# aszepieniec/stark-anatomy

Hardware: AMD Instinct MI355X
Metric: ntt_field_elements_per_sec (higher is better)
Workload: dtype u128; 1 GPU; ntt_fwd_inv_2^20_1gpu; log2n=20, parallelism=single, passes_per_transform=2

## Files before the change

### include/starkcore.h

```cpp
#ifndef STARKCORE_H
#define STARKCORE_H
#include <stdint.h>

#ifdef __cplusplus
extern "C" {
#endif

#define SC_OK 0
#define SC_ERR_HIP (-1)
#define SC_ERR_NOT_POW2 (-2)
#define SC_ERR_ROOT_ORDER (-3)
#define SC_ERR_ROOT_NOT_PRIMITIVE (-4)
#define SC_ERR_DIV_ZERO (-5)
#define SC_ERR_BAD_ARG (-6)
#define SC_ERR_UNSUPPORTED (-7)
#define SC_ERR_NOT_INIT (-8)
#define SC_ERR_TIMEOUT (-9)

typedef struct sc_vec sc_vec_t;
typedef struct sc_merkle sc_merkle_t;
typedef struct sc_merkle_forest sc_merkle_forest_t;
typedef struct sc_later sc_later_t;
typedef struct sc_polytree sc_polytree_t;
typedef struct sc_geodomain sc_geodomain_t;

int sc_device_count(void);
int sc_init(int device);
int sc_shutdown(void);
const char* sc_last_error(void);
int sc_synchronize(void);
int sc_stream(void** stream_out);
int sc_stream_join(void* other_stream);
int sc_set_tuning(const char* key, int value);
int sc_ntt_num_passes(uint64_t n);
int sc_debug_trace(void* d_buf);

int sc_field_selftest(int op, const void* a, const void* b, void* out, uint64_t n);
int sc_field_selftest2(int op, const void* a, const void* b, const void* c, const void* d, void* out, uint32_t* word, uint64_t n);

int sc_vec_alloc(uint64_t n, sc_vec_t** out);
int sc_vec_free(sc_vec_t* v);
int sc_vec_wrap(void* d_elems, uint64_t n, sc_vec_t** out);
uint64_t sc_vec_len(const sc_vec_t* v);
void* sc_vec_ptr(sc_vec_t* v);
int sc_vec_zero(sc_vec_t* v);
int sc_vec_upload(sc_vec_t* v, uint64_t offset, const void* host, uint64_t count);
int sc_vec_download(const sc_vec_t* v, uint64_t offset, void* host, uint64_t count);
int sc_vec_gather(const sc_vec_t* v, const uint64_t* indices, uint64_t k, void* host_out);
int sc_memcpy_dev(void* d_dst, const void* d_src, uint64_t count, void* stream);

int sc_ntt(const void* in, void* out, uint64_t n, const uint64_t root[2], int inverse);
int sc_ntt_dev(const void* d_in, void* d_out, uint64_t n, const uint64_t root[2], int inverse, void* stream);
int sc_ntt_columns_dev(const void* d_in, void* d_out, uint64_t n, uint64_t cols, const uint64_t root[2], int inverse, void* stream);

int sc_ntt_batch_dev(const void* d_in, void* d_out, uint64_t len, uint64_t batch, int kind, const uint64_t root[2], void* stream);
int sc_ntt_batch_ex_dev(const void* d_in, void* d_out, uint64_t len, uint64_t batch, int kind, const uint64_t root[2],
                        const uint64_t outer_root[2], uint64_t outer_order, uint64_t outer_col_base, int outer_scale_ninv, uint64_t chunks, void* stream);
int sc_ntt_rows_t_ld_dev(const void* d_in, void* d_out, uint64_t len, uint64_t batch, const uint64_t root[2], uint64_t chunks, uint64_t out_ld, void* stream);
typedef struct sc_fourstep sc_fourstep_t;
typedef struct { char internal[128]; } sc_rccl_id_t;
int sc_fourstep_create(int log2n, const uint64_t root[2], int rank, int world, sc_fourstep_t** plan);
int sc_fourstep_create_ex(int log2n, const uint64_t root[2], int rank, int world, int log_n1, sc_fourstep_t** plan);
int sc_fourstep_free(sc_fourstep_t* plan);
int sc_fourstep_shape(const sc_fourstep_t* plan, int inverse, uint64_t* rows, uint64_t* cols_total);
int sc_fourstep_cols_dev(const sc_fourstep_t* plan, int inverse, const void* d_src, void* d_send, void* d_recv_diag, void* stream);
int sc_fourstep_rows_dev(const sc_fourstep_t* plan, int inverse, const void* d_recv, void* d_dst, uint64_t block, uint64_t nblocks, int defer_last_pass, void* stream);
int sc_fourstep_rows_finish_dev(const sc_fourstep_t* plan, int inverse, void* d_dst, void* stream);
int sc_comm_unique_id(const char* rccl_path, sc_rccl_id_t* id_out);
int sc_comm_init(const char* rccl_path, const sc_rccl_id_t* id, int rank, int world);
int sc_comm_destroy(void);
int sc_fourstep_run_dev(const sc_fourstep_t* plan, int inverse, const void* d_src, void* d_send, void* d_recv, void* d_dst, uint64_t nblocks, int defer_last_pass,
                        int force_diag_exchange, void* stream);
int sc_ipc_region_create(uint64_t bytes, void** d_region, uint8_t handle_out[64]);
int sc_ipc_region_create_ex(uint64_t bytes, int kind, void** d_region, uint8_t handle_out[64]);
int sc_ipc_region_kind(int* fine_grained);
int sc_ipc_region_open(const uint8_t handle[64], void** d_region);
int sc_ipc_region_close(void* d_region);
int sc_ipc_region_free(void* d_region);
int sc_fourstep_region_bytes(const sc_fourstep_t* plan, uint64_t* bytes);
int sc_fourstep_set_peers(sc_fourstep_t* plan, void* const* regions);
int sc_fourstep_run_direct_dev(sc_fourstep_t* plan, int inverse, const void* d_src, void* d_dst, void* stream);
int sc_fourstep_direct_status(const sc_fourstep_t* plan, uint64_t* timed_out_epoch);
int sc_twiddle_matrix_dev(void* d_data, uint64_t rows, uint64_t cols, uint64_t row_base, uint64_t col_base, const uint64_t root[2], uint64_t order,
                          const uint64_t scale[2], void* stream);

int sc_coset_evaluate(const void* coeffs, uint64_t m, const uint64_t offset[2], const uint64_t generator[2], uint64_t order, void* out);
int sc_coset_evaluate_dev(const void* d_coeffs, uint64_t m, const uint64_t offset[2], const uint64_t generator[2], uint64_t order, void* d_out, void* stream);
// ... 130 lines not shown
```

### stark-anatomy_amd/csrc/core.h

```cpp
#pragma once
#include <hip/hip_runtime.h>
#include <dlfcn.h>
#include <cstdio>
#include <cstdlib>
#include <cstring>
#include <algorithm>
#include <atomic>
#include <chrono>
#include <cerrno>
#include <thread>
#include <sys/random.h>
#include <deque>
#include <functional>
#include <future>
#include <map>
#include <mutex>
#include <string>
#include <tuple>
#include <vector>

#pragma GCC visibility push(default)
#include "../../include/starkcore.h"
#pragma GCC visibility pop
#include "ntt_plan.h"
// ... 43 lines not shown

struct PlanKey {
    int logn;
    uint64_t lo, hi;
    bool operator<(const PlanKey& o) const { return std::tie(logn, lo, hi) < std::tie(o.logn, o.lo, o.hi); }
};
struct PlanTables {
    Fe* mt = nullptr;
    int mt_log = 0;
    Fe* tl = nullptr;
    Fe* th = nullptr;
    Fe* th_ninv = nullptr;
    struct Direct { int logA, logR; bool scaled; Fe* d; };
    std::vector<Direct> direct;
    uint64_t last_use = 0;
};
struct OuterKey {
    uint64_t lo, hi, order, len, batch, col_base;
    int ninv;
    bool operator<(const OuterKey& o) const { return std::tie(lo, hi, order, len, batch, col_base, ninv) < std::tie(o.lo, o.hi, o.order, o.len, o.batch, o.col_base, o.ninv); }
};
struct OuterTable {
    Fe* d = nullptr;
    uint64_t last_use = 0;
};
struct PowKey {
    uint64_t lo, hi, hi_count;
    bool operator<(const PowKey& o) const { return std::tie(lo, hi, hi_count) < std::tie(o.lo, o.hi, o.hi_count); }
};
struct PowTables {
    Fe* lo = nullptr;
    Fe* hi = nullptr;
    uint64_t last_use = 0;
};

struct Ctx {
    bool init = false;
    int device = -1;
    hipStream_t stream = nullptr;
    std::string err;
    NttTuning tuning;
    std::map<PlanKey, PlanTables> plans;
    std::map<PowKey, PowTables> pows;
    std::map<OuterKey, OuterTable> outers;
    uint64_t tick = 0;
    bool foreign_streams = false;
    int small_divisor_direct = 1;
    int div_cols_launch_log = 26;
    int div_cols_chunk = 0;
    std::vector<hipStream_t> seen_streams;
    DevBuf scratch[8];
    std::map<hipStream_t, DevBuf> ntt_work;
    std::map<hipStream_t, DevBuf> ntt_flags;
    int fast_fixups = 1;
    int num_cus = 256;
    int xcd_remap = 1;
    int fixed_shapes = 1;
    int prio_balance = -1;
    int wave_local = 1;
    unsigned long long* trace = nullptr;
    int forest_four_lane_wgs = 256;
    int merkle_big_nlev = 2;
    int fri_tail = -1;
    int fri_tail_stall = -1;
    size_t verify_stage_bytes = 64ull << 20;
    uint8_t* root_slots = nullptr;
    uint8_t* later_words = nullptr;
    uint64_t root_seq = 0;
    std::vector<int> free_root_slots;
};
constexpr int ROOT_SLOTS = 256;
constexpr size_t ROOT_SLOT_BYTES = 128;
constexpr size_t LATER_WORD_BYTES = 128;
constexpr long SPIN_POLLS = 40000000;

struct PendingFree {
    void* p;
    size_t bytes;
    std::vector<hipEvent_t> evs;
};
#define HIPCHK(expr)                                                                                          \
    do {                                                                                                      \
        hipError_t _e = (expr);                                                                               \
        if (_e != hipSuccess) return fail(SC_ERR_HIP, std::string(#expr) + ": " + hipGetErrorString(_e));     \
    } while (0)

#define SCCHK(expr)              \
    do {                         \
        int _rc = (expr);        \
        if (_rc != SC_OK) return _rc; \
    } while (0)

struct NttOpts {
    uint64_t in_limit = ~0ull;
    const PowTables* coset = nullptr;
    uint32_t cols = 1;
    uint64_t col_stride_in = 0;
};
constexpr uint64_t COLS_ELEMS_PER_LAUNCH = 1ull << 26;
constexpr uint64_t SMALL_DIVISOR = 8;

constexpr uint64_t FUSE_MAX_W = 1ull << 17;

enum BuildMode { BUILD_SYNC = 0, BUILD_ASYNC = 1, BUILD_NOROOT = 2 };

extern Ctx g;
// ... 129 lines not shown
```

### stark-anatomy_amd/csrc/core.hip

```cpp
#include "core.h"


template <int LOGE> struct PassThreads { static constexpr int value = LOGE >= 4 ? 256 : (LOGE == 3 ? 512 : 1024); };

template <int LOGE>
__global__ void __launch_bounds__(PassThreads<LOGE>::value) ntt_pass_kernel(const PassParams P, uint32_t ntiles, int xcd_remap) {
    extern __shared__ __attribute__((aligned(16))) unsigned char smem_raw[];
    Fe* lds = reinterpret_cast<Fe*>(smem_raw);
    uint32_t wg = blockIdx.x, colbits = 0;
    if (P.col_enable) { colbits = (wg >> P.col_tiles_log) << P.col_tiles_log; wg -= colbits; }
    uint32_t tile = wg;
    if (xcd_remap) tile = (wg & 7u) * (ntiles >> 3) + (wg >> 3);
    tile |= colbits;
    Fe* tw = lds + (1u << (P.logR + P.logC));
    tile_twiddles_to_lds(P, P.logR, threadIdx.x, blockDim.x, tw);
    __syncthreads();
    const int nrounds = (P.logR + LOGE - 1) / LOGE;
    int sh = P.logR;
    for (int r = 0; r < nrounds; ++r) {
        const int s = (r == 0) ? (P.logR - LOGE * (nrounds - 1)) : LOGE;
        sh -= s;
        ntt_round_dispatch<LOGE>(P, s, sh, r == 0, tile, threadIdx.x, lds, tw);
        if (r + 1 < nrounds) __syncthreads();
    }
// ... 8 lines not shown
    if constexpr (TRACE) {
        if (P.trace) {
            trow = P.trace + ((size_t)blockIdx.x * (blockDim.x >> 6) + (threadIdx.x >> 6)) * TRACE_STAMPS;
            if ((threadIdx.x & 63u) == 0) { trow[0] = __builtin_amdgcn_s_memtime(); trow[15] = __builtin_amdgcn_s_memrealtime(); }
        }
    }
    uint32_t wg = blockIdx.x, colbits = 0;
    if (P.col_enable) { colbits = (wg >> P.col_tiles_log) << P.col_tiles_log; wg -= colbits; }
    uint32_t tile = wg;
    if (xcd_remap) tile = (wg & 7u) * (ntiles >> 3) + (wg >> 3);
    tile |= colbits;
    Fe* tw = lds + (1u << (GLR + GLC));
    auto stamp = [&](int i) {
        if constexpr (TRACE) {
            if (trow) {
                if (i == 2) __builtin_amdgcn_s_waitcnt(0);
                if ((threadIdx.x & 63u) == 0 && i < 13) trow[i] = __builtin_amdgcn_s_memtime();
            }
        }
    };
    auto sync = [] { __syncthreads(); };
    auto wsync = [] { __builtin_amdgcn_fence(__ATOMIC_RELEASE, "wavefront"); __builtin_amdgcn_wave_barrier(); __builtin_amdgcn_fence(__ATOMIC_ACQUIRE, "wavefront"); };
    FixedRounds<LOGE, GLR, GLC, 0, ALT>::run(P, tile, threadIdx.x, lds, tw, sync, wsync, stamp, wave_local != 0);
    if constexpr (TRACE) {
        if (trow && (threadIdx.x & 63u) == 0) { __builtin_amdgcn_s_waitcnt(0); trow[14] = __builtin_amdgcn_s_memtime(); trow[13] = __builtin_amdgcn_s_memrealtime(); }
    }
}

template <int GLR, int GLC>
__device__ __forceinline__ uint32_t fixed8_tile(const PassParams& P, uint32_t index, uint32_t ntiles, int xcd_remap) {
    uint32_t wg = index, colbits = 0;
    if (P.col_enable) { colbits = (wg >> P.col_tiles_log) << P.col_tiles_log; wg -= colbits; }
    uint32_t tile = wg;
    if (xcd_remap) tile = (wg & 7u) * (ntiles >> 3) + (wg >> 3);
    return tile | colbits;
}
template <int GLR, int GLC>
__global__ void __launch_bounds__(1 << (GLR + GLC - 3)) __attribute__((amdgpu_waves_per_eu(4)))
ntt_pass_kernel_fixed8(const PassParams P, uint32_t ntiles, int xcd_remap, int wave_local, uint32_t* flags) {
    extern __shared__ __attribute__((aligned(16))) unsigned char smem_raw[];
    Fe* lds = reinterpret_cast<Fe*>(smem_raw);
    const uint32_t tile = fixed8_tile<GLR, GLC>(P, blockIdx.x, ntiles, xcd_remap);
    Fe* tw = lds + (1u << (GLR + GLC));
    auto stamp = [](int) {};
    auto sync = [] { __syncthreads(); };
    auto wsync = [] { __builtin_amdgcn_fence(__ATOMIC_RELEASE, "wavefront"); __builtin_amdgcn_wave_barrier(); __builtin_amdgcn_fence(__ATOMIC_ACQUIRE, "wavefront"); };
    rare_t rare = 0;
    FixedRounds<3, GLR, GLC, 0, false, true>::run(P, tile, threadIdx.x, lds, tw, sync, wsync, stamp, wave_local != 0, rare);
    if (rare_any(rare)) Round<3, 3, GLR, GLC>::store_word_at(flags + blockIdx.x, 0u, 1u);
}

template <int GLR, int GLC>
__global__ void __launch_bounds__(1 << (GLR + GLC - 3)) __attribute__((amdgpu_waves_per_eu(4)))
ntt_pass_redo8_kernel(const PassParams P, uint32_t ntiles, int xcd_remap, int wave_local, uint32_t* flags, int all) {
    extern __shared__ __attribute__((aligned(16))) unsigned char smem_raw[];
    if (!all && flags[blockIdx.x] == 0) return;
    Fe* lds = reinterpret_cast<Fe*>(smem_raw);
    Fe* tw = lds + (1u << (GLR + GLC));
    auto stamp = [](int) {};
    auto sync = [] { __syncthreads(); };
    auto wsync = [] { __builtin_amdgcn_fence(__ATOMIC_RELEASE, "wavefront"); __builtin_amdgcn_wave_barrier(); __builtin_amdgcn_fence(__ATOMIC_ACQUIRE, "wavefront"); };
    FixedRounds<3, GLR, GLC, 0, false>::run(P, fixed8_tile<GLR, GLC>(P, blockIdx.x, ntiles, xcd_remap), threadIdx.x, lds, tw, sync, wsync, stamp, wave_local != 0);
    if (!all) __syncthreads();
    if (threadIdx.x == 0) flags[blockIdx.x] = 0;
}

__global__ void __launch_bounds__(256) pow_table_kernel(Fe* out, uint64_t count, Fe base_m, uint64_t step, Fe scale_m) {
    uint64_t i = (uint64_t)blockIdx.x * blockDim.x + threadIdx.x;
    if (i < count) out[i] = pow_table_entry(base_m, i, step, scale_m);
}

__global__ void __launch_bounds__(256) twiddle_table_kernel(Fe* out, int logB, uint64_t count, uint64_t scale_exp, const Fe* __restrict__ tl, const Fe* __restrict__ th) {
    uint64_t i = (uint64_t)blockIdx.x * blockDim.x + threadIdx.x;
    if (i >= count) return;
    uint64_t k = i >> logB, b = i & ((1ull << logB) - 1);
    out[i] = pow2level(tl, th, b * k * scale_exp);
}

__global__ void __launch_bounds__(256) pointwise_mul_kernel(const Fe* __restrict__ a, const Fe* __restrict__ b, Fe* __restrict__ out, uint64_t n) {
    uint64_t i = (uint64_t)blockIdx.x * blockDim.x + threadIdx.x;
    if (i < n) out[i] = fe_mul(a[i], b[i]);
}

template <int K>
__global__ void __launch_bounds__(256) pointwise_div_kernel(const Fe* __restrict__ a, const Fe* __restrict__ b, Fe* __restrict__ out, uint64_t n, uint32_t* flag) {
    const uint64_t nthreads = (uint64_t)gridDim.x * blockDim.x;
    const uint64_t t = (uint64_t)blockIdx.x * blockDim.x + threadIdx.x;
    Fe bm[K], pre[K];
    Fe acc = fe_mont_one();
    bool zero = false;
#pragma unroll
    for (int k = 0; k < K; ++k) {
        uint64_t i = t + (uint64_t)k * nthreads;
        Fe v = (i < n) ? b[i] : fe_one();
        zero |= fe_is_zero(v);
        bm[k] = to_mont(v);
        pre[k] = acc;
        acc = mont_mul(acc, bm[k]);
    }
    if (zero) atomicOr(flag, 1u);
    Fe inv = mont_inv(acc);
#pragma unroll
    for (int k = K - 1; k >= 0; --k) {
        uint64_t i = t + (uint64_t)k * nthreads;
        Fe ik = mont_mul(inv, pre[k]);
        inv = mont_mul(inv, bm[k]);
        if (i < n) out[i] = mont_mul(a[i], ik);
    }
}

__global__ void __launch_bounds__(256) short_poly_coset_kernel(const Fe* __restrict__ b, uint32_t nb, Fe off_m, const Fe* __restrict__ tl, const Fe* __restrict__ th, Fe* __restrict__ out, uint64_t order) {
    const uint64_t i = (uint64_t)blockIdx.x * blockDim.x + threadIdx.x;
    if (i >= order) return;
    const Fe x_m = mont_mul(off_m, pow2level(tl, th, i));
    Fe acc = b[nb - 1];
    for (uint32_t k = nb - 1; k-- > 0;) acc = fe_add(mont_mul(acc, x_m), b[k]);
    out[i] = acc;
// ... 401 lines not shown
    it->second.last_use = g.tick;
    *out = &it->second;
    return SC_OK;
}

int get_pow(Fe base, uint64_t count, hipStream_t st, PowTables** out) {
    uint64_t hi_count = (count >> 12) + 1;
    uint64_t hc = 1; while (hc < hi_count) hc <<= 1;
    PowKey key{base.lo, base.hi, hc};
    auto it = g.pows.find(key);
    ++g.tick;
    if (it == g.pows.end()) {
        SCCHK(evict_tables(g.pows, POW_CAP, [](PowTables& t) { hipFree(t.lo); hipFree(t.hi); }));
        Fe bm = to_mont(base);
        PowTables t;
        SCCHK(build_pow_table(&t.lo, 4096, bm, 1, fe_mont_one(), st));
        SCCHK(build_pow_table(&t.hi, hc, bm, 4096, fe_mont_one(), st));
        HIPCHK(hipStreamSynchronize(st));
        it = g.pows.emplace(key, t).first;
    }
    it->second.last_use = g.tick;
    *out = &it->second;
    return SC_OK;
}

int direct_twiddles(PlanTables* pt, const NttPlanDesc& d, int i, bool scaled, hipStream_t st, const Fe** out) {
    const DirectTable t = direct_table(d, i, scaled);
    *out = nullptr;
    if (t.logR + t.logB > g.tuning.direct_tw_max_log) return SC_OK;
    for (const PlanTables::Direct& e : pt->direct)
        if (e.logA == t.logA && e.logR == t.logR && e.scaled == t.scaled) { *out = e.d; return SC_OK; }
    const uint64_t count = 1ull << (t.logR + t.logB);
    Fe* p;
    HIPCHK(hipMalloc((void**)&p, count * sizeof(Fe)));
    pt->direct.push_back({t.logA, t.logR, t.scaled, p});
    hipLaunchKernelGGL(twiddle_table_kernel, dim3((unsigned)((count + 255) / 256)), dim3(256), 0, st, p, t.logB, count, 1ull << t.logA,
                       pt->tl, t.scaled ? pt->th_ninv : pt->th);
    HIPCHK(hipGetLastError());
    HIPCHK(hipStreamSynchronize(st));
    *out = p;
    return SC_OK;
}

int plan_batched_direct(NttPlanDesc& d, BatchKind kind, int loglen, int logbatch, PlanTables* pt, const Fe* in, Fe* work, Fe* out, BatchExtras ex, hipStream_t st, bool* ok) {
    const NttTables tb = tables_of(*pt);
    *ok = plan_batched(d, kind, loglen, logbatch, tb, in, work, out, g.tuning, ex);
    if (!*ok || d.npasses != 2) return SC_OK;
    SCCHK(direct_twiddles(pt, d, 0, false, st, &ex.inner_twd));
    if (ex.inner_twd) *ok = plan_batched(d, kind, loglen, logbatch, tb, in, work, out, g.tuning, ex);
    return SC_OK;
}

int pass_flags(hipStream_t st, uint32_t nwg, uint32_t** out) {
    DevBuf& b = g.ntt_flags[st];
    const void* before = b.p;
    const size_t had = b.bytes;
    void* p;
    SCCHK(grow_buffer(b, (size_t)nwg * sizeof(uint32_t), &p));
    if (p != before || b.bytes != had) HIPCHK(hipMemsetAsync(p, 0, b.bytes, st));
    *out = (uint32_t*)p;
    return SC_OK;
}

template <int LOGE>
int launch_pass(const NttPassDesc& pd, hipStream_t st) {
    int remap = (g.xcd_remap && pd.ntiles >= 16 && (pd.ntiles & 7u) == 0) ? 1 : 0;
    const PassKernel k = pass_kernel(pd, g.fixed_shapes != 0);
    if constexpr (LOGE == 2) {
        if (k.kind == PK_FIXED4) {
            const int lr = pd.p.logR, lc = pd.p.logC;
#define SC_LAUNCH_FIXED(LR, LC, TR, ALT) \
    hipLaunchKernelGGL((ntt_pass_kernel_fixed<2, LR, LC, TR, ALT>), dim3(pd.ntiles * pd.cols), dim3(pd.threads), pd.lds_bytes, st, pd.p, pd.ntiles, remap, g.wave_local)
#define SC_FIXED(LR, LC)                                                          \
            if (lr == LR && lc == LC) {                                           \
                if (k.trace) SC_LAUNCH_FIXED(LR, LC, true, false);                \
                else if (k.alt) SC_LAUNCH_FIXED(LR, LC, false, true);             \
                else SC_LAUNCH_FIXED(LR, LC, false, false);                       \
                return SC_OK;                                                     \
            }
            SC_FIXED4_SHAPES(SC_FIXED)
#undef SC_FIXED
        }
    }
    if constexpr (LOGE == 3) {
        if (k.kind == PK_FIXED8) {
            const int lr = pd.p.logR, lc = pd.p.logC;
            const uint32_t nwg = pd.ntiles * pd.cols;
            const bool fast = g.fast_fixups != 0 && fast_pass_ok(pd.p) && !pass_in_place(pd);
            const int all = (!fast || g.fast_fixups == 2) ? 1 : 0;
            uint32_t* flags;
            SCCHK(pass_flags(st, nwg, &flags));
#define SC_FIXED8(LR, LC)                                                                                                                                   \
            if (lr == LR && lc == LC) {                                                                                                                     \
                if (fast) hipLaunchKernelGGL((ntt_pass_kernel_fixed8<LR, LC>), dim3(nwg), dim3(pd.threads), pd.lds_bytes, st, pd.p, pd.ntiles, remap, g.wave_local, flags); \
                hipLaunchKernelGGL((ntt_pass_redo8_kernel<LR, LC>), dim3(nwg), dim3(pd.threads), pd.lds_bytes, st, pd.p, pd.ntiles, remap, g.wave_local, flags, all); \
                return SC_OK;                                                                                                                               \
            }
            SC_FIXED8_SHAPES(SC_FIXED8)
#undef SC_FIXED8
        }
    }
    hipLaunchKernelGGL(ntt_pass_kernel<LOGE>, dim3(pd.ntiles * pd.cols), dim3(pd.threads), pd.lds_bytes, st, pd.p, pd.ntiles, remap);
    return SC_OK;
}

int run_plan(NttPlanDesc& d, hipStream_t st) {
    size_t trace_off = 0;
    for (int i = 0; i < d.npasses; ++i) {
        d.pass[i].p.prio_balance = pass_prio_balance(d.pass[i], g.prio_balance, g.num_cus);
        d.pass[i].p.trace = g.trace ? g.trace + trace_off : nullptr;
        trace_off += (size_t)d.pass[i].ntiles * d.pass[i].cols * (d.pass[i].threads >> 6) * TRACE_STAMPS;
        switch (d.pass[i].loge) {
            case 1: SCCHK(launch_pass<1>(d.pass[i], st)); break;
            case 2: SCCHK(launch_pass<2>(d.pass[i], st)); break;
            case 3: SCCHK(launch_pass<3>(d.pass[i], st)); break;
            case 4: SCCHK(launch_pass<4>(d.pass[i], st)); break;
            default: return fail(SC_ERR_UNSUPPORTED, "bad loge");
        }
        HIPCHK(hipGetLastError());
    }
    return SC_OK;
}

int ntt_device(const Fe* d_in, Fe* d_out, int logn, Fe root, bool inverse_scale, const NttOpts& o, hipStream_t st) {
    PlanTables* pt;
    SCCHK(get_plan(root, logn, inverse_scale, st, &pt));
    const uint64_t n = 1ull << logn;
    const int m = plan_num_passes(logn, g.tuning);
    NttTables tb = tables_of(*pt);
    tb.th_scaled = (inverse_scale && m > 1) ? pt->th_ninv : nullptr;
    NttIo io;
    io.in = d_in; io.out = d_out; io.in_limit = o.in_limit; io.cols = o.cols; io.col_stride_in = o.col_stride_in;
    if (m > 1) { void* w; SCCHK(grow_buffer(g.ntt_work[st], n * o.cols * sizeof(Fe), &w)); io.work = (Fe*)w; }
    if (o.coset) { io.ol = o.coset->lo; io.oh = o.coset->hi; }
    if (inverse_scale && m == 1) { io.scale_last = true; io.scale = mont_inv(to_mont(Fe{n, 0})); }
    NttPlanDesc d;
    if (!plan_ntt(d, logn, tb, io, g.tuning)) return fail(SC_ERR_UNSUPPORTED, "unsupported transform length");
    if (d.npasses > 1) {
        bool any = false;
        for (int i = 0; i + 1 < d.npasses; ++i) {
            SCCHK(direct_twiddles(pt, d, i, inverse_scale, st, &tb.twd[i]));
            any |= tb.twd[i] != nullptr;
        }
        if (any && !plan_ntt(d, logn, tb, io, g.tuning)) return fail(SC_ERR_UNSUPPORTED, "unsupported transform length");
    }
    return run_plan(d, st);
}

// ... 131 lines not shown
        e = hipStreamSynchronize(h->st);
        landed = e == hipSuccess && __atomic_load_n(host + 8, __ATOMIC_ACQUIRE) == h->seq;
        if (e == hipSuccess && !landed) e = hipErrorUnknown;
    }
    if (landed) memcpy(words, (const void*)host, 64);
    g.free_root_slots.push_back(h->slot);
    delete h;
    if (!landed) return fail(SC_ERR_HIP, hipGetErrorString(e));
    return SC_OK;
}

int gather_device(const Fe* v, const uint64_t* d_idx, uint64_t k, Fe* d_out, hipStream_t st) {
    hipLaunchKernelGGL(gather_kernel, dim3((unsigned)((k + 255) / 256)), dim3(256), 0, st, v, d_idx, k, d_out);
    HIPCHK(hipGetLastError());
    return SC_OK;
}

int evict_outer_tables() { return evict_tables(g.outers, (size_t)16, [](OuterTable& t) { hipFree(t.d); }); }

}


extern "C" {

int sc_device_count(void) {
    int n = 0;
    if (hipGetDeviceCount(&n) != hipSuccess) return 0;
    return n;
}

int sc_init(int device) {
    std::lock_guard<std::mutex> lk(g_mu);
    if (g.init && (device < 0 || device == g.device)) return SC_OK;
    if (g.init) return fail(SC_ERR_BAD_ARG, "already initialised on another device");
    if (device >= 0) { char buf[16]; snprintf(buf, sizeof buf, "%d", device); setenv("STARKCORE_DEVICE", buf, 1); }
    return ensure_init();
}

int sc_shutdown(void) {
    std::lock_guard<std::mutex> lk(g_mu);
    if (g_rand_worker.valid()) { g_rand_worker.get(); g_rand_prefetched = 0; }
    if (!g.init) return SC_OK;
    hipDeviceSynchronize();
    reap_pending(true);
    for (hipEvent_t e : g_event_pool) (void)hipEventDestroy(e);
    g_event_pool.clear();
    free_plans();
    pool_clear();
    for (auto& b : g.scratch) { if (b.p) hipFree(b.p); b = DevBuf{}; }
    for (auto& kv : g.ntt_work) if (kv.second.p) hipFree(kv.second.p);
    g.ntt_work.clear();
    for (auto& kv : g.ntt_flags) if (kv.second.p) hipFree(kv.second.p);
    g.ntt_flags.clear();
    if (g.later_words) hipFree(g.later_words);
    g.later_words = nullptr;
    if (g.stream) hipStreamDestroy(g.stream);
    g.stream = nullptr;
    g.seen_streams.clear();
    g.foreign_streams = false;
    g.init = false;
    return SC_OK;
}

const char* sc_last_error(void) { return g.err.c_str(); }

int sc_synchronize(void) {
    std::lock_guard<std::mutex> lk(g_mu);
    SCCHK(ensure_init());
    HIPCHK(hipStreamSynchronize(g.stream));
    return SC_OK;
}

int sc_stream(void** stream_out) {
    std::lock_guard<std::mutex> lk(g_mu);
    SCCHK(ensure_init());
    if (!stream_out) return fail(SC_ERR_BAD_ARG, "null argument");
    *stream_out = (void*)g.stream;
    return SC_OK;
}

int sc_stream_join(void* other) {
    std::lock_guard<std::mutex> lk(g_mu);
    SCCHK(ensure_init());
    hipStream_t o = (hipStream_t)other;
    if (o == g.stream) return SC_OK;
    (void)pick_stream(other);
    hipEvent_t a = event_get(), b = event_get();
    if (!a || !b) { if (a) g_event_pool.push_back(a); if (b) g_event_pool.push_back(b); HIPCHK(hipStreamSynchronize(o)); HIPCHK(hipStreamSynchronize(g.stream)); return SC_OK; }
    hipError_t e = hipEventRecord(a, o);
    if (e == hipSuccess) e = hipStreamWaitEvent(g.stream, a, 0);
    if (e == hipSuccess) e = hipEventRecord(b, g.stream);
    if (e == hipSuccess) e = hipStreamWaitEvent(o, b, 0);
    g_event_pool.push_back(a);
    g_event_pool.push_back(b);
    if (e != hipSuccess) return fail(SC_ERR_HIP, hipGetErrorString(e));
    return SC_OK;
}

int sc_set_tuning(const char* key, int value) {
    std::lock_guard<std::mutex> lk(g_mu);
    std::string k(key ? key : "");
    if (k == "max_tile_log") g.tuning.max_tile_log = value;
    else if (k == "loge") g.tuning.loge = value;
    else if (k == "max_col_log") g.tuning.max_col_log = value;
    else if (k == "min_tiles_log") g.tuning.min_tiles_log = value;
    else if (k == "single_pass_max_log") g.tuning.single_pass_max_log = value;
    else if (k == "max_digit_log") g.tuning.max_digit_log = value;
    else if (k == "direct_tw_max_log") g.tuning.direct_tw_max_log = value;
    else if (k == "xcd_remap") g.xcd_remap = value;
    else if (k == "fixed_shapes") g.fixed_shapes = value;
    else if (k == "wave_local") g.wave_local = value;
    else if (k == "fast_fixups") g.fast_fixups = value < 0 ? 0 : (value > 2 ? 2 : value);
    else if (k == "prio_balance") g.prio_balance = value;
    else if (k == "loge_cols") g.tuning.loge_cols = value;
    else if (k == "tw_on_load") g.tuning.tw_on_load = value;
    else if (k == "prune") g.tuning.prune = value;
    else if (k == "merkle_big_nlev") g.merkle_big_nlev = value < 0 ? 0 : (value > 8 ? 8 : value);
    else if (k == "forest_four_lane_wgs") g.forest_four_lane_wgs = value < 0 ? 0 : value;
    else if (k == "fri_tail") g.fri_tail = value ? 1 : 0;
    else if (k == "small_divisor_direct") g.small_divisor_direct = value ? 1 : 0;
    else if (k == "div_cols_chunk") g.div_cols_chunk = value < 0 ? 0 : (value > 65535 ? 65535 : value);
    else if (k == "div_cols_launch_log") g.div_cols_launch_log = value < 1 ? 1 : (value > 26 ? 26 : value);
    else if (k == "verify_stage_kb") g.verify_stage_bytes = (size_t)(value < 16 ? 16 : value) << 10;
    else if (k == "fri_tail_stall") g.fri_tail_stall = value;
    else if (k == "pool_cap_mb") g_pool_cap = (size_t)(value < 0 ? 0 : value) << 20;
    else if (k == "pool_trim") {
        if (g.init) { (void)hipDeviceSynchronize(); reap_pending(true); pool_clear(); }
    }
    else return fail(SC_ERR_BAD_ARG, "unknown tuning key " + k);
    return SC_OK;
}

int sc_ntt_num_passes(uint64_t n) {
    std::lock_guard<std::mutex> lk(g_mu);
    if (n < 2 || !is_pow2(n)) return 0;
    return plan_num_passes(ilog2(n), g.tuning);
}

int sc_debug_trace(void* d_buf) {
    std::lock_guard<std::mutex> lk(g_mu);
    g.trace = (unsigned long long*)d_buf;
    return SC_OK;
}

int sc_vec_alloc(uint64_t n, sc_vec_t** out) {
    std::lock_guard<std::mutex> lk(g_mu);
    SCCHK(ensure_init());
    sc_vec* v = new sc_vec{nullptr, n};
    hipError_t e = pool_alloc((void**)&v->d, (n ? n : 1) * sizeof(Fe));
    if (e != hipSuccess) { delete v; return fail(SC_ERR_HIP, hipGetErrorString(e)); }
    *out = v;
    return SC_OK;
}
int sc_vec_free(sc_vec_t* v) {
    std::lock_guard<std::mutex> lk(g_mu);
    if (!v) return SC_OK;
    if (v->owned) release_after_streams(v->d, (v->n ? v->n : 1) * sizeof(Fe));
    delete v;
    return SC_OK;
}
int sc_vec_wrap(void* d_elems, uint64_t n, sc_vec_t** out) {
    if (!d_elems || !out) return fail(SC_ERR_BAD_ARG, "null argument");
    sc_vec* v = new sc_vec{(Fe*)d_elems, n};
    v->owned = false;
    *out = v;
    return SC_OK;
}
uint64_t sc_vec_len(const sc_vec_t* v) { return v ? v->n : 0; }
void* sc_vec_ptr(sc_vec_t* v) { return v ? v->d : nullptr; }
int sc_vec_zero(sc_vec_t* v) {
    std::lock_guard<std::mutex> lk(g_mu);
    if (!v) return fail(SC_ERR_BAD_ARG, "null vector");
    SCCHK(ensure_init());
    if (v->n) HIPCHK(hipMemsetAsync(v->d, 0, v->n * sizeof(Fe), g.stream));
    return SC_OK;
}
}
namespace sci {
struct SmallPayload { uint64_t w[256]; };
__global__ void __launch_bounds__(256) small_upload_kernel(uint64_t* __restrict__ dst, const SmallPayload p, uint32_t nwords) {
    if (threadIdx.x < nwords) dst[threadIdx.x] = p.w[threadIdx.x];
}
bool upload_small(void* d_dst, const void* host, size_t bytes, hipStream_t st) {
    if (bytes > 4 * sizeof(SmallPayload)) return false;
    const uint8_t* src = (const uint8_t*)host;
    uint64_t* dst = (uint64_t*)d_dst;
    for (size_t left = bytes; left;) {
        const size_t take = left < sizeof(SmallPayload) ? left : sizeof(SmallPayload);
        SmallPayload p;
        p.w[(take - 1) / 8] = 0;
        memcpy(p.w, src, take);
// ... 635 lines not shown
```

### stark-anatomy_amd/starkcore.py

```python
import array
import ctypes
import itertools
import os
from collections.abc import Sequence

_HERE = os.path.dirname(os.path.abspath(__file__))
_LIB_PATH = os.environ.get("STARKCORE_LIB") or os.path.join(_HERE, "libstarkcore.so")

_u64 = ctypes.c_uint64
_vp = ctypes.c_void_p
_int = ctypes.c_int

SC_ERR_NOT_POW2 = -2
SC_ERR_ROOT_ORDER = -3
SC_ERR_ROOT_NOT_PRIMITIVE = -4
SC_ERR_DIV_ZERO = -5
SC_ERR_UNSUPPORTED = -7
SC_ERR_TIMEOUT = -9
FOREST_MAX_LEAVES = 1 << 24

SIGNATURES = {
    "sc_device_count": (_int, []),
    "sc_init": (_int, [_int]),
    "sc_shutdown": (_int, []),
    "sc_last_error": (ctypes.c_char_p, []),
    "sc_synchronize": (_int, []),
    "sc_stream": (_int, [ctypes.POINTER(_vp)]),
    "sc_stream_join": (_int, [_vp]),
    "sc_set_tuning": (_int, [ctypes.c_char_p, _int]),
    "sc_ntt_num_passes": (_int, [_u64]),
    "sc_debug_trace": (_int, [_vp]),
    "sc_field_selftest": (_int, [_int, _vp, _vp, _vp, _u64]),
    "sc_field_selftest2": (_int, [_int, _vp, _vp, _vp, _vp, _vp, _vp, _u64]),
    "sc_vec_alloc": (_int, [_u64, ctypes.POINTER(_vp)]),
    "sc_vec_free": (_int, [_vp]),
    "sc_vec_wrap": (_int, [_vp, _u64, ctypes.POINTER(_vp)]),
    "sc_vec_len": (_u64, [_vp]),
    "sc_vec_ptr": (_vp, [_vp]),
    "sc_vec_zero": (_int, [_vp]),
    "sc_vec_upload": (_int, [_vp, _u64, _vp, _u64]),
    "sc_vec_download": (_int, [_vp, _u64, _vp, _u64]),
    "sc_vec_gather": (_int, [_vp, _vp, _u64, _vp]),
    "sc_memcpy_dev": (_int, [_vp, _vp, _u64, _vp]),
    "sc_sample_bytes_dev": (_int, [_vp, _u64, ctypes.c_uint32, _vp, _vp]),
    "sc_sample_urandom_dev": (_int, [_u64, ctypes.c_uint32, _vp, _vp]),
    "sc_urandom_prefetch": (_int, [_u64, ctypes.c_uint32]),
    "sc_rescue_prime_hash_dev": (_int, [_vp, _u64, _vp, _u64, _vp, _vp]),
    "sc_rescue_prime_trace_dev": (_int, [_vp, _u64, _vp, _u64, _vp, _vp]),
    "sc_ntt": (_int, [_vp, _vp, _u64, _vp, _int]),
    "sc_ntt_dev": (_int, [_vp, _vp, _u64, _vp, _int, _vp]),
    "sc_ntt_columns_dev": (_int, [_vp, _vp, _u64, _u64, _vp, _int, _vp]),
    "sc_ntt_batch_dev": (_int, [_vp, _vp, _u64, _u64, _int, _vp, _vp]),
    "sc_ntt_batch_ex_dev": (_int, [_vp, _vp, _u64, _u64, _int, _vp, _vp, _u64, _u64, _int, _u64, _vp]),
    "sc_ntt_rows_t_ld_dev": (_int, [_vp, _vp, _u64, _u64, _vp, _u64, _u64, _vp]),
    "sc_fourstep_create": (_int, [_int, _vp, _int, _int, ctypes.POINTER(_vp)]),
    "sc_fourstep_create_ex": (_int, [_int, _vp, _int, _int, _int, ctypes.POINTER(_vp)]),
    "sc_ipc_region_create": (_int, [_u64, ctypes.POINTER(_vp), _vp]),
    "sc_ipc_region_create_ex": (_int, [_u64, _int, ctypes.POINTER(_vp), _vp]),
    "sc_ipc_region_open": (_int, [_vp, ctypes.POINTER(_vp)]),
    "sc_ipc_region_kind": (_int, [ctypes.POINTER(_int)]),
    "sc_ipc_region_close": (_int, [_vp]),
    "sc_ipc_region_free": (_int, [_vp]),
    "sc_fourstep_region_bytes": (_int, [_vp, ctypes.POINTER(_u64)]),
    "sc_fourstep_set_peers": (_int, [_vp, _vp]),
    "sc_fourstep_run_direct_dev": (_int, [_vp, _int, _vp, _vp, _vp]),
    "sc_fourstep_direct_status": (_int, [_vp, ctypes.POINTER(_u64)]),
    "sc_fourstep_free": (_int, [_vp]),
    "sc_fourstep_shape": (_int, [_vp, _int, ctypes.POINTER(_u64), ctypes.POINTER(_u64)]),
    "sc_fourstep_cols_dev": (_int, [_vp, _int, _vp, _vp, _vp, _vp]),
    "sc_fourstep_rows_dev": (_int, [_vp, _int, _vp, _vp, _u64, _u64, _int, _vp]),
    "sc_fourstep_rows_finish_dev": (_int, [_vp, _int, _vp, _vp]),
    "sc_comm_unique_id": (_int, [ctypes.c_char_p, _vp]),
    "sc_comm_init": (_int, [ctypes.c_char_p, _vp, _int, _int]),
    "sc_comm_destroy": (_int, []),
    "sc_fourstep_run_dev": (_int, [_vp, _int, _vp, _vp, _vp, _vp, _u64, _int, _int, _vp]),
    "sc_twiddle_matrix_dev": (_int, [_vp, _u64, _u64, _u64, _u64, _vp, _u64, _vp, _vp]),
    "sc_coset_evaluate": (_int, [_vp, _u64, _vp, _vp, _u64, _vp]),
    "sc_coset_evaluate_dev": (_int, [_vp, _u64, _vp, _vp, _u64, _vp, _vp]),
    "sc_coset_evaluate_columns_dev": (_int, [_vp, _u64, _u64, _vp, _vp, _u64, _vp, _vp]),
    "sc_poly_mul": (_int, [_vp, _u64, _vp, _u64, _vp, _u64, _vp, _u64]),
    "sc_coset_divide": (_int, [_vp, _u64, _vp, _u64, _vp, _vp, _u64, _vp, _u64]),
    "sc_coset_divide_dev": (_int, [_vp, _u64, _vp, _u64, _vp, _vp, _u64, _vp, _u64, ctypes.POINTER(_int), _vp]),
    "sc_vec_degree_dev": (_int, [_vp, _u64, ctypes.POINTER(ctypes.c_int64), _vp]),
# ... 64 lines not shown
    "sc_polytree_points": (_u64, [_vp]),
    "sc_polytree_zerofier_dev": (_int, [_vp, _vp, _vp]),
    "sc_polytree_evaluate_dev": (_int, [_vp, _vp, _u64, _vp, _vp, _vp]),
    "sc_polytree_interpolate_dev": (_int, [_vp, _vp, _vp, _vp]),
    "sc_polytree_free": (_int, [_vp]),
    "sc_geodomain_create": (_int, [_vp, _vp, _u64, ctypes.POINTER(_vp), _vp]),
    "sc_geodomain_points": (_u64, [_vp]),
    "sc_geodomain_detect_dev": (_int, [_vp, _u64, _vp, _vp, ctypes.POINTER(_int), _vp]),
    "sc_geodomain_zerofier_dev": (_int, [_vp, _vp, _vp]),
    "sc_geodomain_evaluate_dev": (_int, [_vp, _vp, _u64, _vp, _vp]),
    "sc_geodomain_interpolate_dev": (_int, [_vp, _vp, _vp, _vp]),
    "sc_geodomain_interpolate_columns_dev": (_int, [_vp, _vp, _u64, _u64, _vp, _u64, _vp]),
    "sc_geodomain_free": (_int, [_vp]),
}

_lib = None


def _one_hip_runtime():
    import importlib.util
    import sys
    import warnings
    if "torch" in sys.modules or os.environ.get("STARKCORE_NO_TORCH") == "1":
        return
    try:
        spec = importlib.util.find_spec("torch")
    except (ImportError, ValueError):
        spec = None
    if spec is None or not spec.submodule_search_locations:
        return
    runtime = os.path.join(list(spec.submodule_search_locations)[0], "lib", "libamdhip64.so")
    try:
        if os.path.exists(runtime):
            ctypes.CDLL(runtime, mode=ctypes.RTLD_GLOBAL)
            return
    except OSError as e:
        warnings.warn("starkcore: could not preload torch's HIP runtime (%s); importing torch instead" % e)
    try:
        import torch
    except Exception as e:
        warnings.warn("starkcore: torch is installed but neither its HIP runtime nor torch itself could be loaded (%r); a later "
                      "`import torch` in this process may not see the GPU (set STARKCORE_NO_TORCH=1 to silence)" % (e,))


def lib():
    global _lib
    if _lib is None:
        if not os.path.exists(_LIB_PATH):
            raise RuntimeError("libstarkcore.so not built: run `python -c 'import __graft_entry__ as g; g.build()'` "
                               "or `make -C stark-anatomy_amd/csrc` (the HIP extension is mandatory, there is no CPU fallback)")
        _one_hip_runtime()
        l = ctypes.CDLL(_LIB_PATH)
        for name, (res, args) in SIGNATURES.items():
            fn = getattr(l, name)
            fn.restype, fn.argtypes = res, args
        _lib = l
    return _lib


class StarkCoreError(RuntimeError):
    pass


def _check(rc):
    if rc == 0:
        return
    msg = lib().sc_last_error().decode(errors="replace")
    if rc in (SC_ERR_NOT_POW2, SC_ERR_ROOT_ORDER, SC_ERR_ROOT_NOT_PRIMITIVE, SC_ERR_DIV_ZERO):
        raise AssertionError(msg)
    raise StarkCoreError("starkcore error %d: %s" % (rc, msg))


def device_count():
    return lib().sc_device_count()


def init(device=-1):
    _check(lib().sc_init(device))


def set_tuning(key, value):
    _check(lib().sc_set_tuning(key.encode(), int(value)))


def synchronize():
    _check(lib().sc_synchronize())


def library_stream():
    h = _vp()
    _check(lib().sc_stream(ctypes.byref(h)))
    return int(h.value or 0)


def stream_join(other):
    _check(lib().sc_stream_join(_vp(int(other))))


def pickle_proof(ops, moduli, nfields, modulus_bytes, expect=0):
    import numpy as np
    need = ctypes.c_uint64()
    size = len(ops) + int(expect)
    cap = size + size // 8 + 4096
    out = getattr(_pickle_scratch, "buffer", None)
    if out is None or out.size < cap:
        out = _pickle_scratch.buffer = np.empty(cap + cap // 4, dtype=np.uint8)
    _check(lib().sc_pickle_proof(ops, len(ops), moduli, nfields, modulus_bytes, _vp(out.ctypes.data), out.size, ctypes.byref(need)))
    if need.value > out.size:
        out = _pickle_scratch.buffer = np.empty(need.value + need.value // 4, dtype=np.uint8)
        _check(lib().sc_pickle_proof(ops, len(ops), moduli, nfields, modulus_bytes, _vp(out.ctypes.data), out.size, ctypes.byref(need)))
    return out[:need.value].tobytes()


import threading as _threading
_pickle_scratch = _threading.local()


def fe_bytes(v):
    return int(v).to_bytes(16, "little")


def pack(values):
    values = values if isinstance(values, (list, tuple)) else list(values)
    try:
        return b"".join(map(int.to_bytes, values, itertools.repeat(16), itertools.repeat("little")))
    except TypeError:
        return b"".join(int(v).to_bytes(16, "little") for v in values)


def unpack(buf, count=None):
    if count is None:
        count = len(buf) // 16
    limbs = _limb_struct(count).unpack_from(buf)
    return [lo | (hi << 64) for lo, hi in zip(limbs[0::2], limbs[1::2])]

# ... 711 lines not shown
```

Baseline: 48.77 billion field-elements/s.

## Compact fixup redo launch to scan flags per wave and skip idle tiles

The redo kernel used to launch one workgroup per tile, and each workgroup only read its flag before exiting. It now launches a grid 32x smaller in which each wave ballots over 32 tiles' flags and loops over the flagged ones, so most idle workgroup launches go away. When the fast path is off, a separate exact kernel is launched instead, and flags are no longer allocated for that case. The change also adds a device counter of redone tiles, incremented atomically, plus an API to read it. If many tiles need redoing, they are now serialized within one workgroup.

```diff
diff --git a/include/starkcore.h b/include/starkcore.h
--- a/include/starkcore.h
+++ b/include/starkcore.h
@@ -33,6 +33,7 @@
 int sc_stream_join(void* other_stream);
 int sc_set_tuning(const char* key, int value);
 int sc_ntt_num_passes(uint64_t n);
+int sc_ntt_redone_tiles(uint64_t* out, int reset);
 int sc_debug_trace(void* d_buf);
 
 int sc_field_selftest(int op, const void* a, const void* b, void* out, uint64_t n);
diff --git a/stark-anatomy_amd/csrc/core.h b/stark-anatomy_amd/csrc/core.h
--- a/stark-anatomy_amd/csrc/core.h
+++ b/stark-anatomy_amd/csrc/core.h
@@ -119,6 +119,7 @@
     DevBuf scratch[8];
     std::map<hipStream_t, DevBuf> ntt_work;
     std::map<hipStream_t, DevBuf> ntt_flags;
+    unsigned long long* ntt_redone = nullptr;
     int fast_fixups = 1;
     int num_cus = 256;
     int xcd_remap = 1;
diff --git a/stark-anatomy_amd/csrc/core.hip b/stark-anatomy_amd/csrc/core.hip
--- a/stark-anatomy_amd/csrc/core.hip
+++ b/stark-anatomy_amd/csrc/core.hip
@@ -84,17 +84,44 @@
 
 template <int GLR, int GLC>
 __global__ void __launch_bounds__(1 << (GLR + GLC - 3)) __attribute__((amdgpu_waves_per_eu(4)))
-ntt_pass_redo8_kernel(const PassParams P, uint32_t ntiles, int xcd_remap, int wave_local, uint32_t* flags, int all) {
+ntt_pass_exact8_kernel(const PassParams P, uint32_t ntiles, int xcd_remap, int wave_local) {
     extern __shared__ __attribute__((aligned(16))) unsigned char smem_raw[];
-    if (!all && flags[blockIdx.x] == 0) return;
     Fe* lds = reinterpret_cast<Fe*>(smem_raw);
     Fe* tw = lds + (1u << (GLR + GLC));
     auto stamp = [](int) {};
     auto sync = [] { __syncthreads(); };
     auto wsync = [] { __builtin_amdgcn_fence(__ATOMIC_RELEASE, "wavefront"); __builtin_amdgcn_wave_barrier(); __builtin_amdgcn_fence(__ATOMIC_ACQUIRE, "wavefront"); };
     FixedRounds<3, GLR, GLC, 0, false>::run(P, fixed8_tile<GLR, GLC>(P, blockIdx.x, ntiles, xcd_remap), threadIdx.x, lds, tw, sync, wsync, stamp, wave_local != 0);
-    if (!all) __syncthreads();
-    if (threadIdx.x == 0) flags[blockIdx.x] = 0;
+}
+
+constexpr uint32_t REDO_SPAN = 32;
+template <int GLR, int GLC>
+__global__ void __launch_bounds__(1 << (GLR + GLC - 3)) __attribute__((amdgpu_waves_per_eu(4)))
+ntt_pass_redo8_kernel(const PassParams P, uint32_t ntiles, int xcd_remap, int wave_local, uint32_t* flags, uint32_t nwg, int all, unsigned long long* redone) {
+    extern __shared__ __attribute__((aligned(16))) unsigned char smem_raw[];
+    const uint32_t first = (blockIdx.x & 7u) + 8u * (blockIdx.x >> 3), step = gridDim.x;
+    const uint32_t mine = first + (threadIdx.x & (REDO_SPAN - 1u)) * step;
+    uint32_t f = 0;
+    if (mine < nwg) f = all ? 1u : flags[mine];
+    uint32_t todo = (uint32_t)__ballot(f != 0);
+    if (todo == 0) return;
+    auto stamp = [](int) {};
+    auto sync = [] { __syncthreads(); };
+    auto wsync = [] { __builtin_amdgcn_fence(__ATOMIC_RELEASE, "wavefront"); __builtin_amdgcn_wave_barrier(); __builtin_amdgcn_fence(__ATOMIC_ACQUIRE, "wavefront"); };
+    do {
+        const uint32_t index = first + (uint32_t)__builtin_ctz(todo) * step;
+        todo &= todo - 1u;
+        Fe* lds = reinterpret_cast<Fe*>(smem_raw);
+        Fe* tw = lds + (1u << (GLR + GLC));
+        uint32_t tid = threadIdx.x;
+        auto kp = (const __attribute__((address_space(4))) PassParams*)__builtin_amdgcn_kernarg_segment_ptr();
+        asm volatile("" : "+v"(tid));
+        asm volatile("" : "+s"(kp));
+        const PassParams& Q = *(const PassParams*)kp;
+        FixedRounds<3, GLR, GLC, 0, false>::run(Q, fixed8_tile<GLR, GLC>(Q, index, ntiles, xcd_remap), tid, lds, tw, sync, wsync, stamp, wave_local != 0);
+        __syncthreads();
+        if (threadIdx.x == 0) { flags[index] = 0; atomicAdd(redone, 1ull); }
+    } while (todo);
 }
 
 __global__ void __launch_bounds__(256) pow_table_kernel(Fe* out, uint64_t count, Fe base_m, uint64_t step, Fe scale_m) {
@@ -602,6 +629,11 @@
 }
 
 int pass_flags(hipStream_t st, uint32_t nwg, uint32_t** out) {
+    if (!g.ntt_redone) {
+        HIPCHK(hipMalloc((void**)&g.ntt_redone, sizeof(unsigned long long)));
+        HIPCHK(hipMemset(g.ntt_redone, 0, sizeof(unsigned long long)));
+        HIPCHK(hipDeviceSynchronize());
+    }
     DevBuf& b = g.ntt_flags[st];
     const void* before = b.p;
     const size_t had = b.bytes;
@@ -637,13 +669,16 @@
             const int lr = pd.p.logR, lc = pd.p.logC;
             const uint32_t nwg = pd.ntiles * pd.cols;
             const bool fast = g.fast_fixups != 0 && fast_pass_ok(pd.p) && !pass_in_place(pd);
-            const int all = (!fast || g.fast_fixups == 2) ? 1 : 0;
-            uint32_t* flags;
-            SCCHK(pass_flags(st, nwg, &flags));
+            uint32_t* flags = nullptr;
+            if (fast) SCCHK(pass_flags(st, nwg, &flags));
 #define SC_FIXED8(LR, LC)                                                                                                                                   \
             if (lr == LR && lc == LC) {                                                                                                                     \
-                if (fast) hipLaunchKernelGGL((ntt_pass_kernel_fixed8<LR, LC>), dim3(nwg), dim3(pd.threads), pd.lds_bytes, st, pd.p, pd.ntiles, remap, g.wave_local, flags); \
-                hipLaunchKernelGGL((ntt_pass_redo8_kernel<LR, LC>), dim3(nwg), dim3(pd.threads), pd.lds_bytes, st, pd.p, pd.ntiles, remap, g.wave_local, flags, all); \
+                if (fast) {                                                                                                                                 \
+                    hipLaunchKernelGGL((ntt_pass_kernel_fixed8<LR, LC>), dim3(nwg), dim3(pd.threads), pd.lds_bytes, st, pd.p, pd.ntiles, remap, g.wave_local, flags); \
+                    hipLaunchKernelGGL((ntt_pass_redo8_kernel<LR, LC>), dim3(8 * ((nwg + 8 * REDO_SPAN - 1) / (8 * REDO_SPAN))), dim3(pd.threads), pd.lds_bytes, st, pd.p, pd.ntiles, remap, g.wave_local, flags, nwg, g.fast_fixups == 2 ? 1 : 0, g.ntt_redone); \
+                } else {                                                                                                                                    \
+                    hipLaunchKernelGGL((ntt_pass_exact8_kernel<LR, LC>), dim3(nwg), dim3(pd.threads), pd.lds_bytes, st, pd.p, pd.ntiles, remap, g.wave_local); \
+                }                                                                                                                                           \
                 return SC_OK;                                                                                                                               \
             }
             SC_FIXED8_SHAPES(SC_FIXED8)
@@ -881,6 +916,8 @@
     g.ntt_work.clear();
     for (auto& kv : g.ntt_flags) if (kv.second.p) hipFree(kv.second.p);
     g.ntt_flags.clear();
+    if (g.ntt_redone) hipFree(g.ntt_redone);
+    g.ntt_redone = nullptr;
     if (g.later_words) hipFree(g.later_words);
     g.later_words = nullptr;
     if (g.stream) hipStreamDestroy(g.stream);
@@ -966,6 +1003,20 @@
     return plan_num_passes(ilog2(n), g.tuning);
 }
 
+int sc_ntt_redone_tiles(uint64_t* out, int reset) {
+    std::lock_guard<std::mutex> lk(g_mu);
+    SCCHK(ensure_init());
+    if (!out) return fail(SC_ERR_BAD_ARG, "null argument");
+    HIPCHK(hipDeviceSynchronize());
+    unsigned long long v = 0;
+    if (g.ntt_redone) {
+        HIPCHK(hipMemcpy(&v, g.ntt_redone, sizeof v, hipMemcpyDeviceToHost));
+        if (reset) { HIPCHK(hipMemset(g.ntt_redone, 0, sizeof v)); HIPCHK(hipDeviceSynchronize()); }
+    }
+    *out = v;
+    return SC_OK;
+}
+
 int sc_debug_trace(void* d_buf) {
     std::lock_guard<std::mutex> lk(g_mu);
     g.trace = (unsigned long long*)d_buf;
diff --git a/stark-anatomy_amd/starkcore.py b/stark-anatomy_amd/starkcore.py
--- a/stark-anatomy_amd/starkcore.py
+++ b/stark-anatomy_amd/starkcore.py
@@ -29,6 +29,7 @@
     "sc_stream_join": (_int, [_vp]),
     "sc_set_tuning": (_int, [ctypes.c_char_p, _int]),
     "sc_ntt_num_passes": (_int, [_u64]),
+    "sc_ntt_redone_tiles": (_int, [ctypes.POINTER(_u64), _int]),
     "sc_debug_trace": (_int, [_vp]),
     "sc_field_selftest": (_int, [_int, _vp, _vp, _vp, _u64]),
     "sc_field_selftest2": (_int, [_int, _vp, _vp, _vp, _vp, _vp, _vp, _u64]),
@@ -199,7 +200,12 @@
         _one_hip_runtime()
         l = ctypes.CDLL(_LIB_PATH)
         for name, (res, args) in SIGNATURES.items():
-            fn = getattr(l, name)
+            try:
+                fn = getattr(l, name)
+            except AttributeError:
+                if os.environ.get("STARKCORE_LIB"):
+                    continue
+                raise
             fn.restype, fn.argtypes = res, args
         _lib = l
     return _lib
@@ -228,6 +234,12 @@
 
 def set_tuning(key, value):
     _check(lib().sc_set_tuning(key.encode(), int(value)))
+
+
+def redone_tiles(reset=False):
+    out = _u64(0)
+    _check(lib().sc_ntt_redone_tiles(ctypes.byref(out), 1 if reset else 0))
+    return out.value
 
 
 def synchronize():
```

After: 49.16 billion field-elements/s, median of 6. Within noise of the previous version (+0.8%).
